# hojinYang/spotify_recSys_challenge_2018

Measured on AMD Instinct MI355X. Metric: playlists scored/sec (encode+decode+top-500) at |vocab|~170k, higher is better.
Workload: dtype f32; 1 GPU; untied DAE scoring: encode+decode(all 170000 cols)+top-500 over 140000 track cols, hidden=256, batch=256/GPU (global 256), ids=zipf, b_dec=zipf, BASELINE.json configs[1]; vocab=170000, n_tracks=140000, hidden=256, global_batch=256, k=500, parallelism=1 GPU, streams=3, decode_gate=True, tau_exchange=False

## Files before the change

### include/dae_hip.h

```cpp
#ifndef DAE_HIP_H
#define DAE_HIP_H

#include <stddef.h>
#include <stdint.h>

#ifdef __cplusplus
extern "C" {
#endif

typedef struct dae_ctx dae_ctx;

#define DAE_OK            0
#define DAE_ERR_ARG      -1
#define DAE_ERR_HIP      -2
#define DAE_ERR_NOMEM    -3
#define DAE_ERR_STATE    -4

#define DAE_OUT_SCORE     0
#define DAE_OUT_LOGIT     1

#define DAE_DTYPE_F32     0
#define DAE_DTYPE_BF16    1
#define DAE_DTYPE_BF16_EXACT 2

// ... 49 lines not shown
               float* h_out);


int dae_prepack_decoder(dae_ctx* ctx, const float* W_dec, const float* b_dec,
                        int V, int H, int col_lo, int col_hi, int dtype);

int dae_prepack_decoder_rows(dae_ctx* ctx, const float* W_rows, const float* b_rows, int n_rows, int H, int col_lo,
                             int dtype);

int dae_share_decoder(dae_ctx* dst, const dae_ctx* src, int dtype);

int dae_exact_bounds(dae_ctx* ctx, float* eps_out);

int dae_exact_guard_read(dae_ctx* ctx, int32_t* violations, int32_t* column);
int dae_exact_guard_words(dae_ctx* ctx, const int32_t** words_dev);
int dae_exact_guard_snapshot(dae_ctx* ctx, int32_t* words_out_dev);
int dae_exact_stats_read(dae_ctx* ctx, uint64_t out3[3]);

int dae_set_filter_skip(dae_ctx* ctx, int on);
int dae_filter_skip_read(dae_ctx* ctx, uint64_t out3[3]);
int dae_filter_skip_last(dae_ctx* ctx, int32_t* live_out, int cap, int* n_rg_out);
int dae_tile_bounds_read(dae_ctx* ctx, float* ub_out, int cap_tiles, int* ntiles_out);
int dae_sample_skip_read(dae_ctx* ctx, uint64_t out3[3]);
int dae_live_proof_read(dae_ctx* ctx, uint64_t* groups_proved);
int dae_last_tau_read(dae_ctx* ctx, float* tau_out, int B);

int dae_set_exact_margin(dae_ctx* ctx, float scale);
int dae_set_exact_margin_range(dae_ctx* ctx, int col_from, int col_to, float scale);

int dae_set_exact_audit(dae_ctx* ctx, int every_n, int n_tiles);
int dae_exact_audit_read(dae_ctx* ctx, uint64_t out3[3]);


int dae_decode_dense(dae_ctx* ctx, const float* h, int B, int H, int dtype,
                     int apply_sigmoid, float* out, int64_t ld_out);


int dae_decode_topk(dae_ctx* ctx, const float* h, int B, int H, int dtype,
                    int n_tracks,
                    const int32_t* seed_row_ptr, const int32_t* seed_col,
                    int k, int out_kind,
                    float* out_score, int32_t* out_idx);

int dae_score_topk(dae_ctx* ctx,
                   const int32_t* row_ptr, const int32_t* col, const float* val,
                   const float* W_enc, const float* b_enc, int V, int H, int B, int dtype,
// ... 201 lines not shown
```

### spotify_recsys_challenge_2018_amd/_lib.py

```python
import ctypes
import os

_HERE = os.path.dirname(os.path.abspath(__file__))
LIB_PATH = os.path.join(_HERE, "libdae_hip.so")

DAE_OUT_SCORE, DAE_OUT_LOGIT = 0, 1
DAE_MAX_K, DAE_MAX_K_DEEP = 1024, 4096
DAE_DTYPE_F32, DAE_DTYPE_BF16, DAE_DTYPE_BF16_EXACT = 0, 1, 2
DAE_CAND_CHUNK = 256

EXPORTS = [
    "dae_version", "dae_create", "dae_destroy", "dae_set_stream", "dae_last_error",
    "dae_scratch_bytes", "dae_profile_enable", "dae_profile_read", "dae_profile_kernel", "dae_clock_probe", "dae_last_plan",
    "dae_coo_to_csr", "dae_seeds_from_csr", "dae_train_set_create", "dae_train_set_destroy", "dae_train_batch", "dae_train_set_attach_titles", "dae_train_titles", "dae_encode", "dae_prepack_decoder", "dae_prepack_decoder_rows", "dae_share_decoder", "dae_exact_bounds",
    "dae_exact_guard_read", "dae_exact_guard_words", "dae_exact_guard_snapshot", "dae_exact_stats_read", "dae_set_exact_margin", "dae_set_exact_margin_range", "dae_set_exact_audit", "dae_exact_audit_read",
    "dae_set_filter_skip", "dae_filter_skip_read", "dae_filter_skip_last", "dae_tile_bounds_read", "dae_sample_skip_read", "dae_live_proof_read", "dae_last_tau_read", "dae_decode_dense", "dae_decode_topk",
    "dae_score_topk", "dae_score_topk_begin", "dae_score_topk_finish", "dae_topk_dense", "dae_topk_merge", "dae_set_train_dtype", "dae_train_forward_backward",
    "dae_train_shard_encode", "dae_train_shard_decode", "dae_train_shard_finish", "dae_title_features", "dae_title_prepack_features",
    "dae_mix_scores", "dae_decode_mix_term", "dae_set_score_mix", "dae_mix_topk_exact", "dae_mix_exact_shape_ok", "dae_title_score_exact", "dae_title_score", "dae_row_sums", "dae_mix_weights", "dae_title_loss_backward", "dae_title_loss_backward_cols", "dae_title_conv_backward", "dae_adam_step",
    "dae_adam_rows_begin", "dae_adam_rows_apply", "dae_adam_rows_flush", "dae_set_enc_grad_prezeroed",
    "dae_arm_decoder_adam", "dae_set_decode_gate", "dae_set_overlap_hint",
    "dae_pipeline_create", "dae_pipeline_create_titled", "dae_pipeline_destroy", "dae_pipeline_submit", "dae_pipeline_submit_titled", "dae_pipeline_flush", "dae_pipeline_poll",
    "dae_pipeline_release", "dae_pipeline_stats", "dae_pipeline_exact_margin", "dae_pipeline_times", "dae_pipeline_last_error",
    "dae_rank_metrics", "dae_pipeline_enable_eval", "dae_pipeline_submit_eval", "dae_pipeline_poll_eval",
    "dae_decode_candidates", "dae_score_candidates", "dae_mix_candidates", "dae_rank_candidates",
    "dae_catalogue_create", "dae_catalogue_destroy", "dae_prepack_decoder_catalogue", "dae_score_topk_catalogue",
    "dae_decode_topk_catalogue", "dae_title_score_catalogue", "dae_pipeline_set_catalogue",
]
DAE_PIPE_BUSY = 1

_lib = None


class DaeError(RuntimeError):
    pass


def load():
    global _lib
# ... 26 lines not shown
    lib.dae_seeds_from_csr.argtypes = [vp, vp, vp, c_int, c_int, vp, vp]
    lib.dae_train_set_create.argtypes = [vp, vp, vp, vp, vp, c_int, c_int, c_int, ctypes.POINTER(vp)]
    lib.dae_train_set_destroy.argtypes = [vp]
    lib.dae_train_batch.argtypes = [vp, vp, vp, c_int, c_int, vp, vp, vp, c_int, vp, vp, vp, c_int, vp]
    lib.dae_train_set_attach_titles.argtypes = [vp, vp, c_int, c_int, c_int]
    lib.dae_train_titles.argtypes = [vp, vp, vp, c_int, vp]
    lib.dae_encode.argtypes = [vp, vp, vp, vp, vp, vp, c_int, c_int, c_int, c_f, c_f, c_u32, vp]
    lib.dae_prepack_decoder.argtypes = [vp, vp, vp, c_int, c_int, c_int, c_int, c_int]
    lib.dae_prepack_decoder_rows.argtypes = [vp, vp, vp, c_int, c_int, c_int, c_int]
    lib.dae_share_decoder.argtypes = [vp, vp, c_int]
    lib.dae_exact_bounds.argtypes = [vp, vp]
    lib.dae_exact_guard_read.argtypes = [vp, ctypes.POINTER(ctypes.c_int32), ctypes.POINTER(ctypes.c_int32)]
    lib.dae_exact_guard_words.argtypes = [vp, ctypes.POINTER(vp)]
    lib.dae_exact_guard_snapshot.argtypes = [vp, vp]
    lib.dae_set_exact_margin.argtypes = [vp, c_f]
    lib.dae_exact_stats_read.argtypes = [vp, ctypes.POINTER(ctypes.c_uint64)]
    lib.dae_set_exact_margin_range.argtypes = [vp, c_int, c_int, c_f]
    lib.dae_set_exact_audit.argtypes = [vp, c_int, c_int]
    lib.dae_exact_audit_read.argtypes = [vp, ctypes.POINTER(ctypes.c_uint64)]
    lib.dae_set_filter_skip.argtypes = [vp, c_int]
    lib.dae_filter_skip_read.argtypes = [vp, ctypes.POINTER(ctypes.c_uint64)]
    lib.dae_filter_skip_last.argtypes = [vp, ctypes.POINTER(ctypes.c_int32), c_int, ctypes.POINTER(c_int)]
    lib.dae_sample_skip_read.argtypes = [vp, ctypes.POINTER(ctypes.c_uint64)]
    lib.dae_live_proof_read.argtypes = [vp, ctypes.POINTER(ctypes.c_uint64)]
    lib.dae_last_tau_read.argtypes = [vp, ctypes.c_void_p, c_int]
    lib.dae_tile_bounds_read.argtypes = [vp, vp, c_int, ctypes.POINTER(c_int)]
    lib.dae_decode_dense.argtypes = [vp, vp, c_int, c_int, c_int, c_int, vp, c_i64]
    lib.dae_decode_topk.argtypes = [vp, vp, c_int, c_int, c_int, c_int, vp, vp, c_int, c_int, vp, vp]
    lib.dae_score_topk.argtypes = [vp, vp, vp, vp, vp, vp, c_int, c_int, c_int, c_int, c_int, vp, vp,
                                   c_int, c_int, vp, vp]
    lib.dae_score_topk_begin.argtypes = [vp, vp, vp, vp, vp, vp, c_int, c_int, c_int, c_int, c_int, vp, c_int, vp]
    lib.dae_score_topk_finish.argtypes = [vp, vp, vp, vp, c_int, vp, vp]
    lib.dae_topk_dense.argtypes = [vp, vp, c_i64, c_int, c_int, c_int, vp, vp, c_int, c_int, vp, vp]
    lib.dae_topk_merge.argtypes = [vp, c_int, c_int, c_int, vp, vp, c_int, vp, vp]
    lib.dae_set_train_dtype.argtypes = [vp, c_int]
    lib.dae_set_train_dtype.restype = c_int
    lib.dae_train_forward_backward.argtypes = (
        [vp] + [vp] * 6 + [vp] * 4 + [c_int] * 5 + [c_f, c_f, c_u32, c_f] + [vp] * 5)
    lib.dae_train_shard_encode.argtypes = [vp, vp, vp, vp, vp, c_int, c_int, c_int, c_int, c_f, c_u32, vp]
    lib.dae_train_shard_decode.argtypes = (
        [vp, vp, vp] + [vp] * 3 + [vp] * 3 + [c_int] * 6 + [c_f, c_u32, c_f] + [vp] * 4)
    lib.dae_train_shard_finish.argtypes = (
        [vp, vp] + [vp] * 3 + [vp] * 4 + [c_int] * 5 + [c_f, c_f, c_u32, c_f] + [vp] * 4)
    lib.dae_title_features.argtypes = [vp, vp, c_int, c_int, vp, c_int, c_int, vp, vp, ctypes.POINTER(ctypes.c_int32),
                                       c_int, c_int, c_f, c_u32, vp, c_i64, vp, vp]
    lib.dae_title_prepack_features.argtypes = [vp, vp, c_int, c_int, vp, ctypes.POINTER(ctypes.c_int32), c_int, c_int]
# ... 284 lines not shown
        seen = getattr(self, "_guard_seen", 0)
        self._guard_seen = int(n_bad)
        return int(n_bad) != seen

    def exact_stats_read(self):
        a = (ctypes.c_uint64 * 3)()
        self.check(self.lib.dae_exact_stats_read(self.h, a))
        rows = max(int(a[0]), 1)
        return {"rows": int(a[0]), "candidates_per_row": round(int(a[1]) / rows, 1), "recomputed_per_row": round(int(a[2]) / rows, 1)}

    def set_filter_skip(self, on=True):
        self.check(self.lib.dae_set_filter_skip(self.h, 1 if on else 0))

    def filter_skip_read(self):
        a = (ctypes.c_uint64 * 3)()
        self.check(self.lib.dae_filter_skip_read(self.h, a))
        return {"launches": int(a[0]), "planned": int(a[1]), "live": int(a[2])}

    def sample_skip_read(self):
        a = (ctypes.c_uint64 * 3)()
        self.check(self.lib.dae_sample_skip_read(self.h, a))
        return {"launches": int(a[0]), "planned": int(a[1]), "decoded": int(a[2])}

    def live_proof_read(self):
        a = ctypes.c_uint64(0)
        self.check(self.lib.dae_live_proof_read(self.h, ctypes.byref(a)))
        return int(a.value)

    def last_tau(self, B):
        import numpy as np
        out = np.empty(B, np.float32)
        self.check(self.lib.dae_last_tau_read(self.h, out.ctypes.data_as(ctypes.c_void_p), int(B)))
        return out

    def filter_skip_last(self):
        a, n = (ctypes.c_int32 * 64)(), ctypes.c_int()
        self.check(self.lib.dae_filter_skip_last(self.h, a, 64, ctypes.byref(n)))
        return [int(a[i]) for i in range(min(n.value, 64))]

    def tile_bounds(self):
        import numpy as np
        n = ctypes.c_int()
        self.check(self.lib.dae_tile_bounds_read(self.h, None, 0, ctypes.byref(n)))
        out = np.empty((max(n.value, 1), 2), np.float32)
        self.check(self.lib.dae_tile_bounds_read(self.h, out.ctypes.data_as(ctypes.c_void_p), n.value, ctypes.byref(n)))
        return out[:n.value]
# ... 433 lines not shown
```

### spotify_recsys_challenge_2018_amd/csrc/api.hip

```cpp
#include <stdarg.h>

#include <climits>

#include "dae_internal.h"

thread_local std::string g_dae_create_err;

int dae_fail(dae_ctx* ctx, int code, const char* fmt, ...)
{
    char buf[512];
    va_list ap;
    va_start(ap, fmt);
    vsnprintf(buf, sizeof(buf), fmt, ap);
    va_end(ap);
    if (ctx) ctx->err = buf; else g_dae_create_err = buf;
    return code;
}

int dae_reserve(dae_ctx* ctx, dae_buf& b, size_t bytes)
{
    if (bytes <= b.bytes && b.p) return DAE_OK;
    if (bytes == 0) bytes = 16;
    if (b.p) {
        hipError_t e = hipStreamSynchronize(ctx->stream);
// ... 301 lines not shown
    DAE_HIP_CHECK(ctx, hipMemsetAsync(word, 0, sizeof(h), ctx->stream));
    DAE_HIP_CHECK(ctx, hipStreamSynchronize(ctx->stream));
    *groups_proved = (uint64_t)h;
    return DAE_OK;
}

int dae_sample_skip_read(dae_ctx* ctx, uint64_t out3[3])
{
    if (!ctx) return DAE_ERR_ARG;
    if (!out3) return dae_fail(ctx, DAE_ERR_ARG, "null pointer");
    out3[0] = out3[1] = out3[2] = 0;
    if (!ctx->sskip_stat.p) return DAE_OK;
    unsigned long long slots[DAE_SSKIP_SLOTS];
    DAE_HIP_CHECK(ctx, hipMemcpyAsync(slots, ctx->sskip_stat.p, sizeof(slots), hipMemcpyDeviceToHost, ctx->stream));
    DAE_HIP_CHECK(ctx, hipMemsetAsync(ctx->sskip_stat.p, 0, sizeof(slots), ctx->stream));
    DAE_HIP_CHECK(ctx, hipStreamSynchronize(ctx->stream));
    unsigned long long h = 0;
    for (unsigned long long v : slots) h += v;
    out3[0] = (uint64_t)ctx->sskip_launches; out3[1] = (uint64_t)ctx->sskip_planned; out3[2] = (uint64_t)h;
    ctx->sskip_launches = ctx->sskip_planned = 0;
    return DAE_OK;
}

int dae_last_tau_read(dae_ctx* ctx, float* tau_out, int B)
{
    if (!ctx) return DAE_ERR_ARG;
    if (!tau_out || B < 1) return dae_fail(ctx, DAE_ERR_ARG, "dae_last_tau_read: bad arguments");
    if (!ctx->tau.p || (size_t)B * sizeof(float) > ctx->tau.bytes) return dae_fail(ctx, DAE_ERR_STATE, "no thresholds of %d rows on this context", B);
    DAE_HIP_CHECK(ctx, hipMemcpyAsync(tau_out, ctx->tau.p, (size_t)B * sizeof(float), hipMemcpyDeviceToHost, ctx->stream));
    DAE_HIP_CHECK(ctx, hipStreamSynchronize(ctx->stream));
    return DAE_OK;
}

int dae_filter_skip_last(dae_ctx* ctx, int32_t* live_out, int cap, int* n_rg_out)
{
    if (!ctx) return DAE_ERR_ARG;
    if (!n_rg_out || (cap > 0 && !live_out)) return dae_fail(ctx, DAE_ERR_ARG, "null pointer");
    *n_rg_out = ctx->live_n_rg;
    const int n = ctx->live_n_rg < cap ? ctx->live_n_rg : cap;
    if (n <= 0) return DAE_OK;
    DAE_HIP_CHECK(ctx, hipMemcpyAsync(live_out, ctx->live.p, (size_t)n * sizeof(int32_t), hipMemcpyDeviceToHost, ctx->stream));
    DAE_HIP_CHECK(ctx, hipStreamSynchronize(ctx->stream));
    return DAE_OK;
}

int dae_tile_bounds_read(dae_ctx* ctx, float* ub_out, int cap_tiles, int* ntiles_out)
// ... 302 lines not shown
```

### spotify_recsys_challenge_2018_amd/csrc/dae_internal.h

```cpp
#pragma once
#include <hip/hip_runtime.h>
#include <hip/hip_ext.h>
#include <stdint.h>
#include <stdio.h>
#include <stdlib.h>
#include <string.h>
#include <string>
#include <unordered_set>
#include <vector>

#include "../../include/dae_hip.h"
#include "score_plan.h"
#include "mix_plan.h"
#include "tau_search.h"
#include "empty_proof.h"

constexpr int DAE_TITLE_MAX_SIZES = 8;
constexpr int DAE_VT = 32;
constexpr int DAE_HPAD = 32;
constexpr int DAE_REFINED_CAP = 4096;
constexpr size_t DAE_GUARD_BYTES = 2 * sizeof(int);

struct dae_buf {
    void* p = nullptr;
// ... 83 lines not shown
    dae_buf guard;
    float exact_margin = 1.0f;
    int margin_lo = 0, margin_hi = 0; float margin_scale = 1.0f;
    int audit_every = 64, audit_tiles = 16;
    uint64_t audit_seq = 0, audits_run = 0;
    dae_buf title_y1;
    dae_buf audit_stat;
    dae_buf audit;
    dae_buf mix_fhat;
    dae_buf title_scratch;
    dae_buf title_tab; const float* ttab_emb = nullptr; const float* ttab_w = nullptr; int ttab_nchar = 0, ttab_E = 0, ttab_F = 0,
        ttab_nsizes = 0; int ttab_fs[DAE_TITLE_MAX_SIZES] = {0};
    dae_buf tile_band; long long band_gen = -1; int band_nsamp = 0, band_nbrg = 0, band_waves = 0;
    int filter_skip = 1;
    dae_buf live; int live_n_rg = 0;
    dae_buf live_sync; void* live_sync_zeroed = nullptr; size_t live_sync_zeroed_bytes = 0;
    dae_buf cand_list;
    dae_buf cat_seeds;
    dae_buf skip_stat;
    dae_buf row_d; bool row_d_fresh = false;
    dae_buf samp_tab; long long tab_gen = -1; int tab_nsamp = 0, tab_nbrg = 0, tab_waves = 0, tab_nfilter = -1, tab_nrank = -1;
    dae_buf sskip_stat;
    unsigned long long sskip_launches = 0, sskip_planned = 0;

    bool prof_on = false;
    std::vector<hipEvent_t> prof_ev;
    size_t prof_used = 0;
    bool prof_armed = false;
    std::string prof_kernel;
};

extern thread_local std::string g_dae_create_err;

int dae_fail(dae_ctx* ctx, int code, const char* fmt, ...);
int dae_reserve(dae_ctx* ctx, dae_buf& b, size_t bytes);
int dae_ensure_guard(dae_ctx* ctx);

#define DAE_HIP_CHECK(ctx, expr)                                                              \
    do {                                                                                      \
        hipError_t _e = (expr);                                                               \
        if (_e != hipSuccess)                                                                 \
            return dae_fail((ctx), DAE_ERR_HIP, "%s failed: %s (%s:%d)", #expr,               \
                            hipGetErrorString(_e), __FILE__, __LINE__);                       \
    } while (0)

#define DAE_CHECK_LAUNCH(ctx, name)                                                           \
// ... 109 lines not shown
int dae_launch_tile_band(dae_ctx* ctx, const int* order, int ntiles, int n_samp, int nb_rg, int waves, int* band);
int dae_launch_sample_bounds(dae_ctx* ctx, const dae_packed& pk, const int* list, int n_items, int nb_rg, int waves, int nrank,
                             float* head, float2* ub_out, float* beta_out, int n_beta, int n_filter, float* env_out);
int dae_launch_live_tiles(dae_ctx* ctx, const dae_packed& pk, const dae_rowgeom& g, int B, const int* list, int n_items,
                          const float* tau, int nrank, int* live_cnt, int* live_list, unsigned long long* stat);

struct dae_tileset {
    int n_items;
    int stride;
    int mode;
    const int* list;
};
constexpr int DAE_SSKIP_SLOTS = 2 * DAE_NUM_CU;
constexpr int DAE_SSKIP_PAIRS = DAE_SSKIP_SLOTS / DAE_NUM_XCD;
struct dae_sample_skip {
    const float2* ub;
    const float* beta; int n_beta;
    const float* mu;
    const float* row_d;
    const int32_t* seed_row_ptr; int k;
    unsigned long long* stat;
    unsigned* tab;
    float2* pair;
};
int dae_launch_decode_dense_f32(dae_ctx* ctx, const dae_rowgeom& g, int B, const dae_tileset& ts,
                                int apply_sigmoid, int mask_from_col, float* out, int64_t ld,
                                int fill_pad, int dtype = DAE_DTYPE_F32, float* gmax = nullptr,
                                int64_t ld_gmax = 0, int gmax_per_wave = 0, int bias_sel = 0,
                                const dae_sample_skip* skip = nullptr);
int dae_launch_decode_filter_f32(dae_ctx* ctx, const dae_rowgeom& g, int B, const dae_tileset& ts,
                                 const float* tau, int n_valid_col, uint2* cand, int* cand_cnt,
                                 int cap, int dtype = DAE_DTYPE_F32, int bias_sel = 0, const int* live_cnt = nullptr,
                                 const int* live_list = nullptr);

int dae_launch_decode_scaled_T(dae_ctx* ctx, const dae_rowgeom& g, int B, const dae_tileset& ts, const float* row_scale,
                               float* outT, int64_t ldT, int dtype = DAE_DTYPE_F32);

int dae_launch_decode_loss_f32(dae_ctx* ctx, const dae_rowgeom& g, int B, float inv_n_batch,
                               float* dzT, int64_t ldT, float* loss_part, int dtype = DAE_DTYPE_F32,
                               int dz16 = 0);

int dae_launch_decode_loss_rowmajor(dae_ctx* ctx, const dae_rowgeom& g, int B, int V, int H, const float* W,
                                    const float* bias, const float* h, float inv_n_batch, float* dzT, int64_t ldT,
                                    float* loss_part);

int dae_launch_decode_loss_dh(dae_ctx* ctx, const dae_rowgeom& g, int B, int V, int H, const float* W, const float* bias,
                              const float* h, float inv_n_batch, float* dzT, int64_t ldT, float* loss_part, float* part, int Bpad64);
// ... 183 lines not shown
```

### spotify_recsys_challenge_2018_amd/csrc/decode_generic.hip

```cpp
#include "decode_common.h"

namespace {

template <int RB, int EPI, int GT, int NW, int DT, int HALF = 0>
__global__ __launch_bounds__(NW * 64, HALF ? 2 : NW / 4) void decode_f32_kernel(const dae_decp p)
{
    extern __shared__ __attribute__((aligned(16))) float4 lds4[];
    const int tid = threadIdx.x;
    const int lane = tid & 63;
    const int wave = __builtin_amdgcn_readfirstlane(tid >> 6);
    const int hi = lane >> 5;
    const int j = lane & 31;
    const int G = GT > 0 ? GT : p.G;
    constexpr int R_TILE = RB * 32;

    const int gs = DAE_NUM_XCD * p.n_rg;
    const int q = blockIdx.x / gs, rem = blockIdx.x % gs;
    const int rg = rem / DAE_NUM_XCD;
    const int bir = q * DAE_NUM_XCD + (rem % DAE_NUM_XCD);

    const int n_ws = p.nb_rg * NW;
    const int item0 = dae_sample_slot_item(bir, wave, p.nb_rg);
    const bool has0 = item0 < p.ts.n_items;
    const int tv_cur = tile_of_item(p.ts, has0 ? item0 : 0);
    const int tv_nxt = tile_of_item(p.ts, has0 ? (item0 + n_ws < p.ts.n_items ? item0 + n_ws : item0) : 0);
    const int n_h4 = RB * 64 * G;
    bool skip_w = false;
    if constexpr (HALF) {
        static_assert(RB == 2 && EPI == EPI_GMAX, "half row groups: the threshold sample, 64 rows");
        if (p.sk.ub) {
            int* const sk_live = reinterpret_cast<int*>(lds4 + n_h4);
            const int row = rg * R_TILE + lane;
            const bool real = row < p.B;
            const float4 d4 = real ? reinterpret_cast<const float4*>(p.sk.row_d)[row] : make_float4(0.f, 0.f, 0.f, 0.f);
            int ns = (real && p.sk.seed_row_ptr) ? p.sk.seed_row_ptr[row + 1] - p.sk.seed_row_ptr[row] : 0;
            const int kb = p.sk.k - 1;
            float bw[4];
#pragma unroll
            for (int u = 0; u < 4; ++u) {
                const int idx = kb + lane + 64 * u;
                bw[u] = idx < p.sk.n_beta ? p.sk.beta[idx] : -__builtin_inff();
            }
            const float mu = *p.sk.mu;
            const float2 ub = p.sk.ub[has0 ? item0 : 0];
            const unsigned long long cnt_was = tid == 0 ? p.sk.stat[blockIdx.x] : 0ull;
            float dq = dae_max_nan(dae_max_nan(d4.x, d4.y), dae_max_nan(d4.z, d4.w));
            ns = ns < 0 ? 0 : ns;
#pragma unroll
            for (int sh = 1; sh < 64; sh <<= 1) {
                dq = dae_max_nan(dq, __shfl_xor(dq, sh));
                const int o = __shfl_xor(ns, sh);
                ns = o > ns ? o : ns;
            }
            ns = __builtin_amdgcn_readfirstlane(ns);
            float beta_k;
            if (ns < 256) {
                const float sel = ns < 64 ? bw[0] : ns < 128 ? bw[1] : ns < 192 ? bw[2] : bw[3];
                beta_k = __shfl(sel, ns & 63);
            } else {
                beta_k = kb + ns < p.sk.n_beta ? p.sk.beta[kb + ns] : -__builtin_inff();
            }
            const double pm = (double)dq * (double)mu;
            double xd = (double)beta_k - pm;
            xd -= (fabs((double)beta_k) + fabs(pm)) * 0x1p-48;
            float xf = (float)xd;
            if ((double)xf > xd) xf = nextafterf(xf, -__builtin_inff());
            const float tau_safe = dae_tau_value(dae_okey(xf) >> 16, 1);
            skip_w = has0 && (rg * R_TILE >= p.B || !dae_tile_is_live(ub.x, ub.y, (double)dq, tau_safe));
// ... 12 lines not shown
            if (n_live == 0 && p.sk.tab) return;
            if (n_live == 0) {
                const float4 ninf = make_float4(-__builtin_inff(), -__builtin_inff(), -__builtin_inff(), -__builtin_inff());
                for (int sl = tid; sl < 256 * RB; sl += NW * 64) {
                    const int rb = sl >> 8, s2 = sl & 255;
                    const int r2 = rg * R_TILE + rb * 32 + (s2 & 31);
                    if (r2 < p.B)
                        *reinterpret_cast<float4*>(p.gmax + (size_t)r2 * p.ld_gmax + (size_t)bir * 32 + (s2 >> 5) * 4) = ninf;
                }
                for (int t2 = tid; t2 < NW * 64 * RB && p.out; t2 += NW * 64) {
                    const int rb = t2 / (NW * 64), t3 = t2 % (NW * 64);
                    const int w = t3 >> 6, jj = (t3 & 63) >> 1, half = t3 & 1;
                    const int item_w = w * p.nb_rg + bir;
                    const int r2 = rg * R_TILE + rb * 32 + jj;
                    if (item_w < p.ts.n_items && r2 < p.B) {
                        float* orow = p.out + (size_t)r2 * p.ld + (size_t)item_w * 32 + half * 16;
#pragma unroll
                        for (int q4 = 0; q4 < 4; ++q4) *reinterpret_cast<float4*>(orow + 4 * q4) = ninf;
                    }
                }
                return;
            }
            if (tid == 0) p.sk.stat[blockIdx.x] = cnt_was + (unsigned long long)n_live;
        }
    }
    {
        const float4* src = p.hp + (HALF ? (size_t)(rg >> 1) * (2 * n_h4) : (size_t)rg * n_h4);
        auto sidx = [&](int i) -> int {
            return HALF ? (i / (RB * 64)) * (2 * RB * 64) + (rg & 1) * (RB * 64) + (i % (RB * 64)) : i;
        };
        constexpr int NT = NW * 64;
        int i = tid;
        for (; i + 7 * NT < n_h4; i += 8 * NT) {
            float4 v[8];
#pragma unroll
            for (int u = 0; u < 8; ++u) v[u] = src[sidx(i + u * NT)];
#pragma unroll
            for (int u = 0; u < 8; ++u) lds4[i + u * NT] = v[u];
        }
        for (; i < n_h4; i += NT) lds4[i] = src[sidx(i)];
    }
    int* lcnt = reinterpret_cast<int*>(lds4 + n_h4);
    float* ltau = reinterpret_cast<float*>(lcnt + R_TILE);
    if (EPI == EPI_FILTER) {
        for (int i = tid; i < R_TILE; i += NW * 64) {
            lcnt[i] = 0;
            ltau[i] = rg * R_TILE + i < p.B ? p.tau[rg * R_TILE + i] : __builtin_inff();
        }
    }

    float loss_acc = 0.0f;
    float4 wb0, wb1, wb2, wb3;
    float4 bA[RB], bB[RB];
    constexpr int QR = 16;
    uint4 wq[QR];
    uint4 cb[2][RB];
    uint4 bfrag = make_uint4(0u, 0u, 0u, 0u);
    const uint4 ones = bf16_ones_fragment(hi);
    const uint4* ldsq = reinterpret_cast<const uint4*>(lds4);
    int t_cur = __builtin_amdgcn_readfirstlane(tv_cur), t_nxt = __builtin_amdgcn_readfirstlane(tv_nxt);
    {
        const float4* w0 = p.Wp + (size_t)t_cur * G * 64 + lane;
        if (DT == DT_F32) {
            wb0 = w0[0]; wb1 = w0[64]; wb2 = w0[128]; wb3 = w0[192];
        } else {
            bfrag = p.bias16[(size_t)t_cur * 64 + lane];
            const uint4* q0 = reinterpret_cast<const uint4*>(w0);
#pragma unroll
            for (int u = 0; u < QR; ++u) wq[u] = q0[(size_t)(u < G ? u : G - 1) * 64];
        }
    }
    __syncthreads();

    float tau_r[RB];
    if (EPI == EPI_FILTER) {
#pragma unroll
        for (int rb = 0; rb < RB; ++rb) tau_r[rb] = ltau[rb * 32 + j];
    }
    if (DT == DT_F32) {
#pragma unroll
        for (int rb = 0; rb < RB; ++rb) bA[rb] = lds4[rb * 64 + lane];
    } else {
#pragma unroll
        for (int rb = 0; rb < RB; ++rb) cb[0][rb] = ldsq[rb * 64 + lane];
    }

    auto gmax_round = [&](bool has, int round, const f32x16* accv, const float4* bqv, int tcol0v) {
        float4* xl = HALF ? lds4 : reinterpret_cast<float4*>(lcnt + R_TILE);
        if (p.gmax_per_wave) {
            const size_t slot = ((size_t)round * p.nb_rg * NW + (size_t)wave * p.nb_rg + bir) * 32;
#pragma unroll
            for (int rb = 0; rb < RB; ++rb) {
                const int row = rg * R_TILE + rb * 32 + j;
                if (row >= p.B) continue;
#pragma unroll
                for (int qd = 0; qd < 4; ++qd) {
                    float4 v = make_float4(-__builtin_inff(), -__builtin_inff(), -__builtin_inff(), -__builtin_inff());
                    if (has) {
                        const int lc = tcol0v + 8 * qd;
                        float z[4] = {accv[rb][4 * qd + 0] + bqv[qd].x, accv[rb][4 * qd + 1] + bqv[qd].y,
                                      accv[rb][4 * qd + 2] + bqv[qd].z, accv[rb][4 * qd + 3] + bqv[qd].w};
#pragma unroll
                        for (int e = 0; e < 4; ++e)
                            if (p.col_lo + lc + e >= p.mask_from_col || lc + e >= p.ncols) z[e] = -__builtin_inff();
                        v = make_float4(z[0], z[1], z[2], z[3]);
                    }
                    *reinterpret_cast<float4*>(p.gmax + (size_t)row * p.ld_gmax + slot + 4 * hi + 8 * qd) = v;
                }
            }
            return;
        }
#pragma unroll
        for (int rb = 0; rb < RB; ++rb) {
            __syncthreads();
#pragma unroll
            for (int qd = 0; qd < 4; ++qd) {
                float4 v = make_float4(-__builtin_inff(), -__builtin_inff(), -__builtin_inff(), -__builtin_inff());
                if (has) {
                    const int lc = tcol0v + 8 * qd;
                    float z[4] = {accv[rb][4 * qd + 0] + bqv[qd].x, accv[rb][4 * qd + 1] + bqv[qd].y,
                                  accv[rb][4 * qd + 2] + bqv[qd].z, accv[rb][4 * qd + 3] + bqv[qd].w};
#pragma unroll
                    for (int e = 0; e < 4; ++e)
                        if (p.col_lo + lc + e >= p.mask_from_col || lc + e >= p.ncols) z[e] = -__builtin_inff();
                    v = make_float4(z[0], z[1], z[2], z[3]);
                }
                xl[wave * 256 + (qd * 2 + hi) * 32 + j] = v;
            }
            __syncthreads();
            for (int sl = tid; sl < 256; sl += NW * 64) {
                float4 m = xl[sl];
#pragma unroll
                for (int w = 1; w < NW; ++w) {
                    const float4 o = xl[w * 256 + sl];
                    m = make_float4(fmaxf(m.x, o.x), fmaxf(m.y, o.y), fmaxf(m.z, o.z), fmaxf(m.w, o.w));
                }
                const int row = rg * R_TILE + rb * 32 + (sl & 31);
                if (row < p.B)
                    *reinterpret_cast<float4*>(p.gmax + (size_t)row * p.ld_gmax +
                                               ((size_t)round * p.nb_rg + bir) * 32 + (sl >> 5) * 4) = m;
            }
            for (int t2 = tid; t2 < NW * 64 && p.out; t2 += NW * 64) {
                const int w = t2 >> 6, jj = (t2 & 63) >> 1, half = t2 & 1;
                const int item_w = w * p.nb_rg + bir + round * (p.nb_rg * NW);
                const int row = rg * R_TILE + rb * 32 + jj;
                bool stored = true;
                if constexpr (HALF)
                    if (p.sk.tab) stored = reinterpret_cast<const int*>(lds4 + n_h4)[w] != 0;
                if (item_w < p.ts.n_items && row < p.B && stored) {
                    float* orow = p.out + (size_t)row * p.ld + (size_t)item_w * 32 + half * 16;
#pragma unroll
                    for (int q4 = 0; q4 < 4; ++q4)
                        *reinterpret_cast<float4*>(orow + 4 * q4) = xl[w * 256 + (half * 4 + q4) * 32 + jj];
                }
            }
        }
    };

    for (int item = skip_w ? p.ts.n_items : item0; item < p.ts.n_items; item += n_ws) {
        const int t = t_cur;
        const float4* wp = p.Wp + (size_t)t * G * 64 + lane;
        const int item_n = item + n_ws < p.ts.n_items ? item + n_ws : item;
        const float4* wn = p.Wp + (size_t)t_nxt * G * 64 + lane;
        const int item_nn = item_n + n_ws < p.ts.n_items ? item_n + n_ws : item_n;
        const int t_nn_v = tile_of_item(p.ts, item_nn);

        const float* bp = p.bias + (size_t)t * 32 + 4 * hi;
        float4 bq[4];
#pragma unroll
        for (int qd = 0; qd < 4; ++qd)
            bq[qd] = DT == DT_BF16 ? make_float4(0.f, 0.f, 0.f, 0.f) : *reinterpret_cast<const float4*>(bp + 8 * qd);

        float mixv[(EPI == EPI_GMAX || EPI == EPI_FILTER) ? RB : 1][16];
        if ((EPI == EPI_GMAX || EPI == EPI_FILTER) && p.mixT) {
#pragma unroll
            for (int rb = 0; rb < RB; ++rb) {
                const int row = rg * R_TILE + rb * 32 + j;
#pragma unroll
                for (int e = 0; e < 16; ++e) {
                    const int lc = t * 32 + 4 * hi + (e & 3) + 8 * (e >> 2);
// ... 332 lines not shown
```

### spotify_recsys_challenge_2018_amd/csrc/score.hip

```cpp
#include <climits>

#include "dae_internal.h"

namespace {

thread_local int32_t g_last_plan[8] = {0, 0, 0, 0, 0, 0, 0, 0};

int prof_begin(dae_ctx* ctx)
{
    if (!ctx->prof_on) return DAE_OK;
    if (ctx->prof_used + 2 > ctx->prof_ev.size()) {
        for (int i = 0; i < 2; ++i) {
            hipEvent_t ev;
            DAE_HIP_CHECK(ctx, hipEventCreate(&ev));
            ctx->prof_ev.push_back(ev);
        }
    }
    ctx->prof_armed = true;
    return DAE_OK;
}

dae_rowgeom geom_for(int dtype, int B, int Hp)
{
    return dtype == DAE_DTYPE_F32 ? dae_row_geometry(B, Hp) : dae_row_geometry_bf16(B, Hp);
// ... 161 lines not shown
            }
            order = static_cast<const int*>(ctx->tile_band.p);
        }
    }
    tk.order = order;
    dae_tileset tsA{pl.n_samp, pl.fused ? pl.S : 1, pl.fused ? 3 : 0, order};
    float* gmax = nullptr;
    if (pl.fused || pl.mixed) {
        rc = dae_reserve(ctx, ctx->gmax, (size_t)B * pl.ld_g * sizeof(float));
        if (rc) return rc;
        gmax = static_cast<float*>(ctx->gmax.p);
    }
    dae_sample_skip sk{};
    float* env = nullptr;
    const bool d_fresh = ctx->row_d_fresh;
    ctx->row_d_fresh = false;
    if (pl.sample_skip && ctx->filter_skip) {
        const int n_beta = g.nb_rg * 32 < 4096 ? g.nb_rg * 32 : 4096;
        const void* tab_was = ctx->samp_tab.p;
        rc = dae_reserve(ctx, ctx->samp_tab, (4 + (size_t)2 * pl.n_samp + n_beta + DAE_PROOF_ENV) * sizeof(float));
        if (rc) return rc;
        if (ctx->samp_tab.p != tab_was) ctx->tab_gen = -1;
        if (!ctx->sskip_stat.p) {
            rc = dae_reserve(ctx, ctx->sskip_stat, DAE_SSKIP_SLOTS * (sizeof(unsigned long long) + sizeof(unsigned)) + DAE_SSKIP_PAIRS * sizeof(float2));
            if (rc) return rc;
            DAE_HIP_CHECK(ctx, hipMemsetAsync(ctx->sskip_stat.p, 0, DAE_SSKIP_SLOTS * sizeof(unsigned long long), ctx->stream));
        }
        float* head = static_cast<float*>(ctx->samp_tab.p);
        float2* ub = reinterpret_cast<float2*>(head + 4);
        float* beta = head + 4 + (size_t)2 * pl.n_samp;
        env = beta + n_beta;
        if (ctx->tab_gen != pk->order_gen || ctx->tab_nsamp != pl.n_samp || ctx->tab_nbrg != g.nb_rg || ctx->tab_waves != g.waves ||
            ctx->tab_nfilter != pl.n_filter || ctx->tab_nrank != pl.nrank) {
            rc = dae_launch_sample_bounds(ctx, *pk, order, pl.n_samp, g.nb_rg, g.waves, pl.nrank, head, ub, beta, n_beta, pl.n_filter, env);
            if (rc) return rc;
            ctx->tab_gen = pk->order_gen; ctx->tab_nsamp = pl.n_samp; ctx->tab_nbrg = g.nb_rg; ctx->tab_waves = g.waves;
            ctx->tab_nfilter = pl.n_filter; ctx->tab_nrank = pl.nrank;
        }
        if (d_fresh && 2 * g.grid <= DAE_SSKIP_SLOTS && ctx->row_d.p && ctx->row_d.bytes >= (size_t)g.Bpad * 4 * sizeof(float)) {
            unsigned long long* const stat = static_cast<unsigned long long*>(ctx->sskip_stat.p);
            unsigned* const tab = dae_tau_wave_per_row(B, pl.ld_g, pl.ld_s) ? nullptr : reinterpret_cast<unsigned*>(stat + DAE_SSKIP_SLOTS);
            float2* const pair = reinterpret_cast<float2*>(reinterpret_cast<unsigned*>(stat + DAE_SSKIP_SLOTS) + DAE_SSKIP_SLOTS);
            sk = dae_sample_skip{ub, beta, n_beta, head, static_cast<const float*>(ctx->row_d.p), seed_row_ptr, k, stat, tab, pair};
            ctx->sskip_launches += 1;
            ctx->sskip_planned += (unsigned long long)((B + 63) / 64) * (unsigned long long)pl.n_samp;
        }
    }
    if (!pl.fused) { rc = prof_begin(ctx); if (rc) return rc; }
    rc = dae_launch_decode_dense_f32(ctx, pl.wave_groups ? pl.gA : g, B, tsA, 0, pl.n_valid_col, pl.whole_b ? nullptr : sample, pl.ld_s,
                                     1, pl.dtype, gmax, pl.ld_g, pl.gmax_per_wave, pl.exact ? 1 : 0, sk.ub ? &sk : nullptr);
    if (rc) return rc;
    if (!pl.fused) {
        ctx->prof_armed = false;
        rc = fill_tau_neg_inf(ctx, tau_dst, B);
        tk.valid = rc == DAE_OK;
        return rc;
    }

    const int64_t pstride = pl.ld_s;
    rc = dae_reserve(ctx, ctx->sample_top, ((size_t)g.Bpad * pstride) * sizeof(uint2) + (size_t)g.Bpad * sizeof(int));
    if (rc) return rc;
    tk.sample_cnt = reinterpret_cast<int*>(static_cast<uint2*>(ctx->sample_top.p) + (size_t)g.Bpad * pstride);
    dae_tau_live lv{};
    if (pl.live_in_tau) {
        constexpr size_t n_arrive = 64;
        if ((size_t)g.n_rg > n_arrive) return dae_fail(ctx, DAE_ERR_STATE, "%d row groups in one threshold launch", g.n_rg);
        int* lc; int* ll;
// ... 431 lines not shown
```

Measured before the change: 9.816 million playlists/s.

## Redistribute sampled-tile decode work across idle waves when few waves are live

In the half-row-group threshold-sample decode kernel, waves whose sample tiles were skipped now take over part of the remaining live waves' work. When exactly one of four waves is live, each wave computes a quarter of that tile with 16x16x4 MFMAs. Otherwise idle waves take the second 32-row block of a live wave's tile. Results are merged through LDS into gmax and out. The aim is to cut the critical-path latency of the sample pass when most waves are idle, at the cost of extra LDS traffic, syncs, register pressure and a new share counter.

```diff
diff --git a/include/dae_hip.h b/include/dae_hip.h
--- a/include/dae_hip.h
+++ b/include/dae_hip.h
@@ -95,6 +95,7 @@
 int dae_filter_skip_last(dae_ctx* ctx, int32_t* live_out, int cap, int* n_rg_out);
 int dae_tile_bounds_read(dae_ctx* ctx, float* ub_out, int cap_tiles, int* ntiles_out);
 int dae_sample_skip_read(dae_ctx* ctx, uint64_t out3[3]);
+int dae_sample_share_read(dae_ctx* ctx, uint64_t out2[2]);
 int dae_live_proof_read(dae_ctx* ctx, uint64_t* groups_proved);
 int dae_last_tau_read(dae_ctx* ctx, float* tau_out, int B);
 
diff --git a/spotify_recsys_challenge_2018_amd/_lib.py b/spotify_recsys_challenge_2018_amd/_lib.py
--- a/spotify_recsys_challenge_2018_amd/_lib.py
+++ b/spotify_recsys_challenge_2018_amd/_lib.py
@@ -14,7 +14,7 @@
     "dae_scratch_bytes", "dae_profile_enable", "dae_profile_read", "dae_profile_kernel", "dae_clock_probe", "dae_last_plan",
     "dae_coo_to_csr", "dae_seeds_from_csr", "dae_train_set_create", "dae_train_set_destroy", "dae_train_batch", "dae_train_set_attach_titles", "dae_train_titles", "dae_encode", "dae_prepack_decoder", "dae_prepack_decoder_rows", "dae_share_decoder", "dae_exact_bounds",
     "dae_exact_guard_read", "dae_exact_guard_words", "dae_exact_guard_snapshot", "dae_exact_stats_read", "dae_set_exact_margin", "dae_set_exact_margin_range", "dae_set_exact_audit", "dae_exact_audit_read",
-    "dae_set_filter_skip", "dae_filter_skip_read", "dae_filter_skip_last", "dae_tile_bounds_read", "dae_sample_skip_read", "dae_live_proof_read", "dae_last_tau_read", "dae_decode_dense", "dae_decode_topk",
+    "dae_set_filter_skip", "dae_filter_skip_read", "dae_filter_skip_last", "dae_tile_bounds_read", "dae_sample_skip_read", "dae_sample_share_read", "dae_live_proof_read", "dae_last_tau_read", "dae_decode_dense", "dae_decode_topk",
     "dae_score_topk", "dae_score_topk_begin", "dae_score_topk_finish", "dae_topk_dense", "dae_topk_merge", "dae_set_train_dtype", "dae_train_forward_backward",
     "dae_train_shard_encode", "dae_train_shard_decode", "dae_train_shard_finish", "dae_title_features", "dae_title_prepack_features",
     "dae_mix_scores", "dae_decode_mix_term", "dae_set_score_mix", "dae_mix_topk_exact", "dae_mix_exact_shape_ok", "dae_title_score_exact", "dae_title_score", "dae_row_sums", "dae_mix_weights", "dae_title_loss_backward", "dae_title_loss_backward_cols", "dae_title_conv_backward", "dae_adam_step",
@@ -87,6 +87,7 @@
     lib.dae_filter_skip_read.argtypes = [vp, ctypes.POINTER(ctypes.c_uint64)]
     lib.dae_filter_skip_last.argtypes = [vp, ctypes.POINTER(ctypes.c_int32), c_int, ctypes.POINTER(c_int)]
     lib.dae_sample_skip_read.argtypes = [vp, ctypes.POINTER(ctypes.c_uint64)]
+    lib.dae_sample_share_read.argtypes = [vp, ctypes.POINTER(ctypes.c_uint64)]
     lib.dae_live_proof_read.argtypes = [vp, ctypes.POINTER(ctypes.c_uint64)]
     lib.dae_last_tau_read.argtypes = [vp, ctypes.c_void_p, c_int]
     lib.dae_tile_bounds_read.argtypes = [vp, vp, c_int, ctypes.POINTER(c_int)]
@@ -417,6 +418,11 @@
         self.check(self.lib.dae_sample_skip_read(self.h, a))
         return {"launches": int(a[0]), "planned": int(a[1]), "decoded": int(a[2])}
 
+    def sample_share_read(self):
+        a = (ctypes.c_uint64 * 2)()
+        self.check(self.lib.dae_sample_share_read(self.h, a))
+        return {"launches": int(a[0]), "shared": int(a[1])}
+
     def live_proof_read(self):
         a = ctypes.c_uint64(0)
         self.check(self.lib.dae_live_proof_read(self.h, ctypes.byref(a)))
diff --git a/spotify_recsys_challenge_2018_amd/csrc/api.hip b/spotify_recsys_challenge_2018_amd/csrc/api.hip
--- a/spotify_recsys_challenge_2018_amd/csrc/api.hip
+++ b/spotify_recsys_challenge_2018_amd/csrc/api.hip
@@ -347,6 +347,23 @@
     return DAE_OK;
 }
 
+int dae_sample_share_read(dae_ctx* ctx, uint64_t out2[2])
+{
+    if (!ctx) return DAE_ERR_ARG;
+    if (!out2) return dae_fail(ctx, DAE_ERR_ARG, "null pointer");
+    out2[0] = out2[1] = 0;
+    if (!ctx->sskip_stat.p) return DAE_OK;
+    unsigned slots[DAE_SSKIP_SLOTS];
+    DAE_HIP_CHECK(ctx, hipMemcpyAsync(slots, dae_sshare_words(ctx), sizeof(slots), hipMemcpyDeviceToHost, ctx->stream));
+    DAE_HIP_CHECK(ctx, hipMemsetAsync(dae_sshare_words(ctx), 0, sizeof(slots), ctx->stream));
+    DAE_HIP_CHECK(ctx, hipStreamSynchronize(ctx->stream));
+    unsigned long long h = 0;
+    for (unsigned v : slots) h += v;
+    out2[0] = (uint64_t)ctx->sshare_launches; out2[1] = (uint64_t)h;
+    ctx->sshare_launches = 0;
+    return DAE_OK;
+}
+
 int dae_last_tau_read(dae_ctx* ctx, float* tau_out, int B)
 {
     if (!ctx) return DAE_ERR_ARG;
diff --git a/spotify_recsys_challenge_2018_amd/csrc/dae_internal.h b/spotify_recsys_challenge_2018_amd/csrc/dae_internal.h
--- a/spotify_recsys_challenge_2018_amd/csrc/dae_internal.h
+++ b/spotify_recsys_challenge_2018_amd/csrc/dae_internal.h
@@ -129,6 +129,7 @@
     dae_buf samp_tab; long long tab_gen = -1; int tab_nsamp = 0, tab_nbrg = 0, tab_waves = 0, tab_nfilter = -1, tab_nrank = -1;
     dae_buf sskip_stat;
     unsigned long long sskip_launches = 0, sskip_planned = 0;
+    unsigned long long sshare_launches = 0;
 
     bool prof_on = false;
     std::vector<hipEvent_t> prof_ev;
@@ -284,7 +285,13 @@
     unsigned long long* stat;
     unsigned* tab;
     float2* pair;
-};
+    unsigned* share;
+};
+inline unsigned* dae_sshare_words(dae_ctx* ctx)
+{
+    char* const base = static_cast<char*>(ctx->sskip_stat.p);
+    return reinterpret_cast<unsigned*>(base + DAE_SSKIP_SLOTS * (sizeof(unsigned long long) + sizeof(unsigned)) + DAE_SSKIP_PAIRS * sizeof(float2));
+}
 int dae_launch_decode_dense_f32(dae_ctx* ctx, const dae_rowgeom& g, int B, const dae_tileset& ts,
                                 int apply_sigmoid, int mask_from_col, float* out, int64_t ld,
                                 int fill_pad, int dtype = DAE_DTYPE_F32, float* gmax = nullptr,
diff --git a/spotify_recsys_challenge_2018_amd/csrc/decode_generic.hip b/spotify_recsys_challenge_2018_amd/csrc/decode_generic.hip
--- a/spotify_recsys_challenge_2018_amd/csrc/decode_generic.hip
+++ b/spotify_recsys_challenge_2018_amd/csrc/decode_generic.hip
@@ -1,4 +1,5 @@
 #include "decode_common.h"
+#include "sample_share.h"
 
 namespace {
 
@@ -26,9 +27,17 @@
     const int tv_nxt = tile_of_item(p.ts, has0 ? (item0 + n_ws < p.ts.n_items ? item0 + n_ws : item0) : 0);
     const int n_h4 = RB * 64 * G;
     bool skip_w = false;
+    bool share = false;
+    int sh_owner = -1, sh_rb = 0, sh_quarter = -1;
+    int tv_all[HALF ? NW : 1];
     if constexpr (HALF) {
         static_assert(RB == 2 && EPI == EPI_GMAX, "half row groups: the threshold sample, 64 rows");
         if (p.sk.ub) {
+#pragma unroll
+            for (int w = 0; w < NW; ++w) {
+                const int item_w = dae_sample_slot_item(bir, w, p.nb_rg);
+                tv_all[w] = tile_of_item(p.ts, item_w < p.ts.n_items ? item_w : 0);
+            }
             int* const sk_live = reinterpret_cast<int*>(lds4 + n_h4);
             const int row = rg * R_TILE + lane;
             const bool real = row < p.B;
@@ -44,6 +53,7 @@
             const float mu = *p.sk.mu;
             const float2 ub = p.sk.ub[has0 ? item0 : 0];
             const unsigned long long cnt_was = tid == 0 ? p.sk.stat[blockIdx.x] : 0ull;
+            const unsigned shr_was = tid == 0 ? p.sk.share[blockIdx.x] : 0u;
             float dq = dae_max_nan(dae_max_nan(d4.x, d4.y), dae_max_nan(d4.z, d4.w));
             ns = ns < 0 ? 0 : ns;
 #pragma unroll
@@ -102,6 +112,16 @@
                 return;
             }
             if (tid == 0) p.sk.stat[blockIdx.x] = cnt_was + (unsigned long long)n_live;
+            unsigned vote = 0;
+#pragma unroll
+            for (int w = 0; w < NW; ++w) vote |= (unsigned)sk_live[w] << w;
+            share = dae_sample_shares(vote, NW);
+            if (share) {
+                const dae_share_job job = dae_sample_share_job(vote, wave, NW);
+                sh_owner = job.owner; sh_rb = job.rb; sh_quarter = job.quarter;
+                if (sh_owner >= 0 && sh_rb >= 0 && rg * R_TILE + sh_rb * 32 >= p.B) sh_owner = -1;
+                if (tid == 0) p.sk.share[blockIdx.x] = shr_was + (unsigned)n_live;
+            }
         }
     }
     {
@@ -139,8 +159,20 @@
     const uint4 ones = bf16_ones_fragment(hi);
     const uint4* ldsq = reinterpret_cast<const uint4*>(lds4);
     int t_cur = __builtin_amdgcn_readfirstlane(tv_cur), t_nxt = __builtin_amdgcn_readfirstlane(tv_nxt);
+    if constexpr (HALF) {
+        if (share && sh_owner >= 0) {
+            int t_job = tv_all[0];
+#pragma unroll
+            for (int w = 1; w < NW; ++w) t_job = sh_owner == w ? tv_all[w] : t_job;
+            t_cur = __builtin_amdgcn_readfirstlane(t_job);
+        }
+    }
+    int wl = lane;
+    if constexpr (HALF) {
+        if (sh_quarter >= 0) wl = 16 * (sh_quarter >> 1) + (lane & 15) + 32 * ((lane >> 4) & 1);
+    }
     {
-        const float4* w0 = p.Wp + (size_t)t_cur * G * 64 + lane;
+        const float4* w0 = p.Wp + (size_t)t_cur * G * 64 + wl;
         if (DT == DT_F32) {
             wb0 = w0[0]; wb1 = w0[64]; wb2 = w0[128]; wb3 = w0[192];
         } else {
@@ -165,6 +197,34 @@
         for (int rb = 0; rb < RB; ++rb) cb[0][rb] = ldsq[rb * 64 + lane];
     }
 
+    auto gmax_merge = [&](int rb, int round, const float4* xl) {
+        for (int sl = tid; sl < 256; sl += NW * 64) {
+            float4 m = xl[sl];
+#pragma unroll
+            for (int w = 1; w < NW; ++w) {
+                const float4 o = xl[w * 256 + sl];
+                m = make_float4(fmaxf(m.x, o.x), fmaxf(m.y, o.y), fmaxf(m.z, o.z), fmaxf(m.w, o.w));
+            }
+            const int row = rg * R_TILE + rb * 32 + (sl & 31);
+            if (row < p.B)
+                *reinterpret_cast<float4*>(p.gmax + (size_t)row * p.ld_gmax +
+                                           ((size_t)round * p.nb_rg + bir) * 32 + (sl >> 5) * 4) = m;
+        }
+        for (int t2 = tid; t2 < NW * 64 && p.out; t2 += NW * 64) {
+            const int w = t2 >> 6, jj = (t2 & 63) >> 1, half = t2 & 1;
+            const int item_w = w * p.nb_rg + bir + round * (p.nb_rg * NW);
+            const int row = rg * R_TILE + rb * 32 + jj;
+            bool stored = true;
+            if constexpr (HALF)
+                if (p.sk.tab) stored = reinterpret_cast<const int*>(lds4 + n_h4)[w] != 0;
+            if (item_w < p.ts.n_items && row < p.B && stored) {
+                float* orow = p.out + (size_t)row * p.ld + (size_t)item_w * 32 + half * 16;
+#pragma unroll
+                for (int q4 = 0; q4 < 4; ++q4)
+                    *reinterpret_cast<float4*>(orow + 4 * q4) = xl[w * 256 + (half * 4 + q4) * 32 + jj];
+            }
+        }
+    };
     auto gmax_round = [&](bool has, int round, const f32x16* accv, const float4* bqv, int tcol0v) {
         float4* xl = HALF ? lds4 : reinterpret_cast<float4*>(lcnt + R_TILE);
         if (p.gmax_per_wave) {
@@ -208,34 +268,140 @@
                 xl[wave * 256 + (qd * 2 + hi) * 32 + j] = v;
             }
             __syncthreads();
-            for (int sl = tid; sl < 256; sl += NW * 64) {
-                float4 m = xl[sl];
-#pragma unroll
-                for (int w = 1; w < NW; ++w) {
-                    const float4 o = xl[w * 256 + sl];
-                    m = make_float4(fmaxf(m.x, o.x), fmaxf(m.y, o.y), fmaxf(m.z, o.z), fmaxf(m.w, o.w));
-                }
-                const int row = rg * R_TILE + rb * 32 + (sl & 31);
-                if (row < p.B)
-                    *reinterpret_cast<float4*>(p.gmax + (size_t)row * p.ld_gmax +
-                                               ((size_t)round * p.nb_rg + bir) * 32 + (sl >> 5) * 4) = m;
-            }
-            for (int t2 = tid; t2 < NW * 64 && p.out; t2 += NW * 64) {
-                const int w = t2 >> 6, jj = (t2 & 63) >> 1, half = t2 & 1;
-                const int item_w = w * p.nb_rg + bir + round * (p.nb_rg * NW);
-                const int row = rg * R_TILE + rb * 32 + jj;
-                bool stored = true;
-                if constexpr (HALF)
-                    if (p.sk.tab) stored = reinterpret_cast<const int*>(lds4 + n_h4)[w] != 0;
-                if (item_w < p.ts.n_items && row < p.B && stored) {
-                    float* orow = p.out + (size_t)row * p.ld + (size_t)item_w * 32 + half * 16;
-#pragma unroll
-                    for (int q4 = 0; q4 < 4; ++q4)
-                        *reinterpret_cast<float4*>(orow + 4 * q4) = xl[w * 256 + (half * 4 + q4) * 32 + jj];
-                }
-            }
+            gmax_merge(rb, round, xl);
         }
     };
+
+    if constexpr (HALF) {
+        if (share && sh_quarter >= 0) {
+            typedef float f32x4_t __attribute__((ext_vector_type(4)));
+            const int t = t_cur;
+            const int cb = sh_quarter >> 1, rs = sh_quarter & 1, q4 = lane >> 4, l15 = lane & 15;
+            const bool odd = (q4 >> 1) != 0;
+            const float4* wp = p.Wp + (size_t)t * G * 64 + wl;
+            const float4* hl = lds4 + 16 * rs + l15 + 32 * (q4 & 1);
+            const float4 bq = *reinterpret_cast<const float4*>(p.bias + (size_t)t * 32 + 16 * cb + 4 * q4);
+            f32x4_t c0 = {0.f, 0.f, 0.f, 0.f}, c1 = {0.f, 0.f, 0.f, 0.f};
+            float4 hA0 = hl[0], hA1 = hl[64], hB0, hB1;
+#define DAE_QUARTER_STEP(WB, PF, REFILL, BC0, BC1, BN0, BN1, GNEXT)                            \
+    {                                                                                          \
+        const float4 a = WB;                                                                   \
+        if (REFILL) WB = *(PF);                                                                \
+        BN0 = hl[(size_t)(GNEXT) * (RB * 64)];                                                 \
+        BN1 = hl[(size_t)(GNEXT) * (RB * 64) + 64];                                            \
+        __builtin_amdgcn_sched_barrier(0);                                                     \
+        const float a0 = odd ? a.y : a.x, a1 = odd ? a.w : a.z;                                \
+        c0 = __builtin_amdgcn_mfma_f32_16x16x4f32(a0, odd ? BC0.y : BC0.x, c0, 0, 0, 0);       \
+        c1 = __builtin_amdgcn_mfma_f32_16x16x4f32(a0, odd ? BC1.y : BC1.x, c1, 0, 0, 0);       \
+        c0 = __builtin_amdgcn_mfma_f32_16x16x4f32(a1, odd ? BC0.w : BC0.z, c0, 0, 0, 0);       \
+        c1 = __builtin_amdgcn_mfma_f32_16x16x4f32(a1, odd ? BC1.w : BC1.z, c1, 0, 0, 0);       \
+        __builtin_amdgcn_sched_barrier(0);                                                     \
+    }
+            int g = 0;
+#pragma unroll
+            for (; g < G - 4; g += 4) {
+                const float4* pf = wp + (size_t)(g + 4) * 64;
+                DAE_QUARTER_STEP(wb0, pf,       true, hA0, hA1, hB0, hB1, g + 1)
+                DAE_QUARTER_STEP(wb1, pf + 64,  true, hB0, hB1, hA0, hA1, g + 2)
+                DAE_QUARTER_STEP(wb2, pf + 128, true, hA0, hA1, hB0, hB1, g + 3)
+                DAE_QUARTER_STEP(wb3, pf + 192, true, hB0, hB1, hA0, hA1, g + 4)
+            }
+            DAE_QUARTER_STEP(wb0, wp, false, hA0, hA1, hB0, hB1, g + 1)
+            DAE_QUARTER_STEP(wb1, wp, false, hB0, hB1, hA0, hA1, g + 2)
+            DAE_QUARTER_STEP(wb2, wp, false, hA0, hA1, hB0, hB1, g + 3)
+            DAE_QUARTER_STEP(wb3, wp, false, hB0, hB1, hA0, hA1, 0)
+#undef DAE_QUARTER_STEP
+            float4* xl = lds4;
+            const int lc = t * 32 + 16 * cb + 4 * q4;
+            const float4 ninf = make_float4(-__builtin_inff(), -__builtin_inff(), -__builtin_inff(), -__builtin_inff());
+#pragma unroll
+            for (int rb = 0; rb < RB; ++rb) {
+                __syncthreads();
+                const f32x4_t c = rb ? c1 : c0;
+                float z[4] = {c[0] + bq.x, c[1] + bq.y, c[2] + bq.z, c[3] + bq.w};
+#pragma unroll
+                for (int e = 0; e < 4; ++e)
+                    if (p.col_lo + lc + e >= p.mask_from_col || lc + e >= p.ncols) z[e] = -__builtin_inff();
+                xl[sh_owner * 256 + (4 * cb + q4) * 32 + 16 * rs + l15] = make_float4(z[0], z[1], z[2], z[3]);
+                if (rb == 0 && wave != sh_owner) {
+#pragma unroll
+                    for (int qd = 0; qd < 4; ++qd) xl[wave * 256 + (qd * 2 + hi) * 32 + j] = ninf;
+                }
+                __syncthreads();
+                gmax_merge(rb, 0, xl);
+            }
+            return;
+        }
+        if (share) {
+            const bool job = sh_owner >= 0;
+            const int t = t_cur;
+            const float4* wp = p.Wp + (size_t)t * G * 64 + lane;
+            const float* bp = p.bias + (size_t)t * 32 + 4 * hi;
+            float4 bq[4];
+#pragma unroll
+            for (int qd = 0; qd < 4; ++qd) bq[qd] = *reinterpret_cast<const float4*>(bp + 8 * qd);
+            f32x16 acc1;
+#pragma unroll
+            for (int e = 0; e < 16; ++e) acc1[e] = 0.0f;
+            if (job) {
+                const float4* hl = lds4 + sh_rb * 64 + lane;
+                float4 hA = sh_rb ? bA[1] : bA[0], hB;
+#define DAE_SHARE_STEP(WB, PF, REFILL, BC, BN, GNEXT)                                          \
+    {                                                                                          \
+        const float4 a = WB;                                                                   \
+        if (REFILL) WB = *(PF);                                                                \
+        BN = hl[(size_t)(GNEXT) * (RB * 64)];                                                  \
+        __builtin_amdgcn_sched_barrier(0);                                                     \
+        acc1 = __builtin_amdgcn_mfma_f32_32x32x2f32(a.x, BC.x, acc1, 0, 0, 0);                 \
+        acc1 = __builtin_amdgcn_mfma_f32_32x32x2f32(a.y, BC.y, acc1, 0, 0, 0);                 \
+        acc1 = __builtin_amdgcn_mfma_f32_32x32x2f32(a.z, BC.z, acc1, 0, 0, 0);                 \
+        acc1 = __builtin_amdgcn_mfma_f32_32x32x2f32(a.w, BC.w, acc1, 0, 0, 0);                 \
+        __builtin_amdgcn_sched_barrier(0);                                                     \
+    }
+                int g = 0;
+#pragma unroll
+                for (; g < G - 4; g += 4) {
+                    const float4* pf = wp + (size_t)(g + 4) * 64;
+                    DAE_SHARE_STEP(wb0, pf,       true, hA, hB, g + 1)
+                    DAE_SHARE_STEP(wb1, pf + 64,  true, hB, hA, g + 2)
+                    DAE_SHARE_STEP(wb2, pf + 128, true, hA, hB, g + 3)
+                    DAE_SHARE_STEP(wb3, pf + 192, true, hB, hA, g + 4)
+                }
+                DAE_SHARE_STEP(wb0, wp, false, hA, hB, g + 1)
+                DAE_SHARE_STEP(wb1, wp, false, hB, hA, g + 2)
+                DAE_SHARE_STEP(wb2, wp, false, hA, hB, g + 3)
+                DAE_SHARE_STEP(wb3, wp, false, hB, hA, 0)
+#undef DAE_SHARE_STEP
+            }
+            const int tcol0 = t * 32 + 4 * hi;
+            float4* xl = lds4;
+#pragma unroll
+            for (int rb = 0; rb < RB; ++rb) {
+                __syncthreads();
+                const bool vals = job && sh_rb == rb;
+                if (rb == 0 || vals) {
+                    const int sw = vals ? sh_owner : wave;
+#pragma unroll
+                    for (int qd = 0; qd < 4; ++qd) {
+                        float4 v = make_float4(-__builtin_inff(), -__builtin_inff(), -__builtin_inff(), -__builtin_inff());
+                        if (vals) {
+                            const int lc = tcol0 + 8 * qd;
+                            float z[4] = {acc1[4 * qd + 0] + bq[qd].x, acc1[4 * qd + 1] + bq[qd].y,
+                                          acc1[4 * qd + 2] + bq[qd].z, acc1[4 * qd + 3] + bq[qd].w};
+#pragma unroll
+                            for (int e = 0; e < 4; ++e)
+                                if (p.col_lo + lc + e >= p.mask_from_col || lc + e >= p.ncols) z[e] = -__builtin_inff();
+                            v = make_float4(z[0], z[1], z[2], z[3]);
+                        }
+                        xl[sw * 256 + (qd * 2 + hi) * 32 + j] = v;
+                    }
+                }
+                __syncthreads();
+                gmax_merge(rb, 0, xl);
+            }
+            return;
+        }
+    }
 
     for (int item = skip_w ? p.ts.n_items : item0; item < p.ts.n_items; item += n_ws) {
         const int t = t_cur;
diff --git a/spotify_recsys_challenge_2018_amd/csrc/sample_share.h b/spotify_recsys_challenge_2018_amd/csrc/sample_share.h
--- /dev/null
+++ b/spotify_recsys_challenge_2018_amd/csrc/sample_share.h
@@ -0,0 +1,43 @@
+#pragma once
+#include "tau_search.h"
+
+struct dae_share_job {
+    int owner;
+    int rb;
+    int quarter;
+};
+
+DAE_HD int dae_share_popcount(unsigned vote, int nw)
+{
+    int n = 0;
+    for (int w = 0; w < nw; ++w) n += (int)((vote >> w) & 1u);
+    return n;
+}
+
+DAE_HD bool dae_sample_shares(unsigned vote, int nw)
+{
+    const int n_live = dae_share_popcount(vote, nw);
+    return n_live >= 1 && 2 * n_live <= nw;
+}
+DAE_HD bool dae_sample_shares_quarters(unsigned vote, int nw) { return nw == 4 && dae_share_popcount(vote, nw) == 1; }
+
+DAE_HD dae_share_job dae_sample_share_job(unsigned vote, int wave, int nw)
+{
+    const bool live = ((vote >> wave) & 1u) != 0;
+    if (!dae_sample_shares(vote, nw)) return dae_share_job{live ? wave : -1, -1, -1};
+    if (dae_sample_shares_quarters(vote, nw)) {
+        int owner = 0;
+        for (int w = 0; w < nw; ++w) owner = ((vote >> w) & 1u) ? w : owner;
+        return dae_share_job{owner, -1, wave};
+    }
+    if (live) return dae_share_job{wave, 0, -1};
+    int rank = 0;
+    for (int w = 0; w < wave; ++w) rank += (int)(((vote >> w) & 1u) == 0);
+    int owner = -1;
+    for (int w = 0, seen = 0; w < nw; ++w)
+        if ((vote >> w) & 1u) {
+            if (seen == rank) owner = w;
+            ++seen;
+        }
+    return dae_share_job{owner, owner >= 0 ? 1 : -1, -1};
+}
diff --git a/spotify_recsys_challenge_2018_amd/csrc/score.hip b/spotify_recsys_challenge_2018_amd/csrc/score.hip
--- a/spotify_recsys_challenge_2018_amd/csrc/score.hip
+++ b/spotify_recsys_challenge_2018_amd/csrc/score.hip
@@ -207,9 +207,10 @@
         if (rc) return rc;
         if (ctx->samp_tab.p != tab_was) ctx->tab_gen = -1;
         if (!ctx->sskip_stat.p) {
-            rc = dae_reserve(ctx, ctx->sskip_stat, DAE_SSKIP_SLOTS * (sizeof(unsigned long long) + sizeof(unsigned)) + DAE_SSKIP_PAIRS * sizeof(float2));
+            rc = dae_reserve(ctx, ctx->sskip_stat, DAE_SSKIP_SLOTS * (sizeof(unsigned long long) + 2 * sizeof(unsigned)) + DAE_SSKIP_PAIRS * sizeof(float2));
             if (rc) return rc;
             DAE_HIP_CHECK(ctx, hipMemsetAsync(ctx->sskip_stat.p, 0, DAE_SSKIP_SLOTS * sizeof(unsigned long long), ctx->stream));
+            DAE_HIP_CHECK(ctx, hipMemsetAsync(dae_sshare_words(ctx), 0, DAE_SSKIP_SLOTS * sizeof(unsigned), ctx->stream));
         }
         float* head = static_cast<float*>(ctx->samp_tab.p);
         float2* ub = reinterpret_cast<float2*>(head + 4);
@@ -226,8 +227,9 @@
             unsigned long long* const stat = static_cast<unsigned long long*>(ctx->sskip_stat.p);
             unsigned* const tab = dae_tau_wave_per_row(B, pl.ld_g, pl.ld_s) ? nullptr : reinterpret_cast<unsigned*>(stat + DAE_SSKIP_SLOTS);
             float2* const pair = reinterpret_cast<float2*>(reinterpret_cast<unsigned*>(stat + DAE_SSKIP_SLOTS) + DAE_SSKIP_SLOTS);
-            sk = dae_sample_skip{ub, beta, n_beta, head, static_cast<const float*>(ctx->row_d.p), seed_row_ptr, k, stat, tab, pair};
+            sk = dae_sample_skip{ub, beta, n_beta, head, static_cast<const float*>(ctx->row_d.p), seed_row_ptr, k, stat, tab, pair, dae_sshare_words(ctx)};
             ctx->sskip_launches += 1;
+            ctx->sshare_launches += 1;
             ctx->sskip_planned += (unsigned long long)((B + 63) / 64) * (unsigned long long)pl.n_samp;
         }
     }
```

After: 8.373 million playlists/s. 0.853x the previous value.
